# voidstrike/FPSG

Hardware: AMD Instinct MI355X
Metric: episodes/sec (+ Chamfer-kernel HBM GB/s in roofline.hbm), 2048-pt clouds, 224x224 images; episode = fwd + Chamfer + bwd, step = E episodes + all-reduce + Adam (higher is better)
Workload: dtype f32

## Files before the change

### fpsg_amd/_hip.py

```python
from __future__ import annotations

import ctypes
import os
import threading

import torch

_HERE = os.path.dirname(os.path.abspath(__file__))
LIB_PATH = os.environ.get("FPSG_HIP_LIB") or os.path.join(_HERE, "libfpsg_hip.so")

_c_f32p = ctypes.c_void_p
_c_i32p = ctypes.c_void_p
_c_int = ctypes.c_int
_c_stream = ctypes.c_void_p

SIGNATURES = {
    "fpsg_version": [],
    "fpsg_last_error": [],
    "fpsg_chamfer_fwd": [_c_f32p, _c_f32p, _c_int, _c_int, _c_int,
                         _c_f32p, _c_i32p, _c_f32p, _c_i32p, _c_stream],
    "fpsg_chamfer_bwd": [_c_f32p, _c_f32p, _c_i32p, _c_i32p, _c_f32p, _c_f32p,
                         _c_int, _c_int, _c_int, _c_f32p, _c_f32p, _c_stream],
    "fpsg_chamfer_losses": [_c_f32p, _c_f32p, _c_int, _c_int, _c_int, _c_int, ctypes.c_float, ctypes.c_float, _c_f32p,
                            _c_stream],
# ... 54 lines not shown
                         _c_int, _c_int, _c_int, _c_int, _c_f32p, _c_f32p, _c_f32p, _c_f32p, _c_f32p, _c_stream],
    "fpsg_bn_act_rows_fwd": [_c_f32p, _c_int, ctypes.POINTER(ctypes.c_int), ctypes.POINTER(ctypes.c_int), _c_int,
                             _c_f32p, _c_f32p, _c_f32p, _c_int, ctypes.c_float, _c_int, ctypes.c_float, _c_f32p,
                             _c_f32p, _c_f32p, _c_stream],
    "fpsg_bn_act_rows_bwd": [_c_f32p, _c_int, ctypes.POINTER(ctypes.c_int), ctypes.POINTER(ctypes.c_int), _c_int,
                             _c_f32p, _c_f32p, _c_f32p, _c_int, _c_int, ctypes.c_float, _c_f32p, _c_f32p, _c_f32p,
                             _c_f32p, _c_stream],
    "fpsg_bn_workspace_floats": [_c_int, _c_int, _c_int],
    "fpsg_bn_act_fwd": [_c_f32p, _c_f32p, _c_f32p, _c_f32p, _c_f32p, _c_f32p, ctypes.c_float, _c_int, _c_int, _c_int, _c_int,
                        ctypes.c_float, _c_int, ctypes.c_float, _c_f32p, _c_f32p, _c_f32p, _c_f32p, _c_f32p,
                        _c_stream],
    "fpsg_bn_act_bwd": [_c_f32p, _c_f32p, _c_f32p, _c_f32p, _c_int, _c_int, _c_int, _c_int, _c_int,
                        ctypes.c_float, _c_f32p, _c_f32p, _c_f32p, _c_f32p, _c_f32p, _c_f32p, _c_stream],
    "fpsg_bn_act_bwd_coef": [_c_f32p, _c_f32p, _c_f32p, _c_f32p, _c_int, _c_int, _c_int, _c_int, _c_int, ctypes.c_float,
                             _c_f32p, _c_f32p, _c_f32p, _c_f32p, _c_stream],
    "fpsg_bn_act_bwd_parts": [_c_f32p, _c_f32p, _c_f32p, _c_f32p, _c_int, _c_int, _c_int, _c_int, _c_int,
                        ctypes.c_float, _c_f32p, _c_f32p, _c_f32p, _c_f32p, _c_f32p, _c_f32p, _c_f32p, _c_int, _c_stream],
    "fpsg_bn_pool_workspace_floats": [_c_int, _c_int, _c_int, _c_int],
    "fpsg_bn_act_pool_fwd": [_c_f32p, _c_f32p, _c_f32p, _c_f32p, _c_f32p, _c_f32p, ctypes.c_float, _c_int, _c_int, _c_int, _c_int,
                             _c_int, ctypes.c_float, _c_int, ctypes.c_float, _c_f32p, _c_f32p, _c_f32p, _c_f32p,
                             _c_f32p, _c_f32p, _c_int, _c_stream],
    "fpsg_bn_act_pool_bwd": [_c_f32p, _c_f32p, _c_f32p, _c_f32p, _c_int, _c_int, _c_int, _c_int, _c_int, _c_int,
                             ctypes.c_float, _c_f32p, _c_f32p, _c_f32p, _c_f32p, _c_f32p, _c_f32p, _c_stream],
    "fpsg_bn_max_workspace_floats": [_c_int, _c_int, _c_int],
    "fpsg_bn_max_dz_offset": [_c_int, _c_int, _c_int],
    "fpsg_bn_act_max_fwd": [_c_f32p, _c_f32p, _c_f32p, _c_f32p, _c_f32p, _c_f32p, ctypes.c_float, _c_int, _c_int, _c_int, _c_int,
                            ctypes.c_float, _c_int, ctypes.c_float, _c_f32p, _c_i32p, _c_f32p, _c_f32p, _c_f32p,
                            _c_f32p, _c_stream],
    "fpsg_bn_act_max_bwd": [_c_f32p, _c_f32p, _c_f32p, _c_i32p, _c_f32p, _c_int, _c_int, _c_int, _c_int, _c_int,
                            ctypes.c_float, _c_f32p, _c_f32p, _c_f32p, _c_f32p, _c_f32p, _c_f32p, _c_stream],
# ... 17 lines not shown
    "fpsg_wino_output_transform_bwd_stats": [_c_int, _c_f32p, _c_int, _c_int, _c_int, _c_int, _c_f32p, _c_f32p, _c_f32p,
                                             _c_f32p, _c_f32p, ctypes.c_long, _c_stream],
    "fpsg_wino_filter_transform_batch": [ctypes.c_void_p, _c_int, ctypes.c_long, _c_stream],
    "fpsg_wino_filter_grad_transform": [_c_int, _c_f32p, _c_int, _c_int, _c_f32p, _c_stream],
    "fpsg_wino_conv_fused": [_c_f32p, _c_f32p, _c_int, _c_int, _c_int, _c_int, _c_int, _c_f32p, _c_stream],
    "fpsg_wino_input_transform_act": [_c_int, _c_f32p, _c_f32p, _c_f32p, _c_int, _c_int, _c_int, _c_int, _c_f32p, ctypes.c_long,
                                      _c_stream],
    "fpsg_wino_conv_fused_act": [_c_f32p, _c_f32p, _c_f32p, _c_f32p, _c_int, _c_int, _c_int, _c_int, _c_int, _c_f32p,
                                 _c_stream],
    "fpsg_wino_dw_fused_workspace_floats": [_c_int, _c_int, _c_int, _c_int],
    "fpsg_wino_dw_fused": [_c_f32p, _c_f32p, _c_f32p, _c_f32p, _c_int, _c_int, _c_int, _c_int, _c_int, _c_f32p, _c_f32p,
                           _c_stream],
    "fpsg_wino_conv_fused_parts": [_c_int, _c_int, _c_int, _c_int],
    "fpsg_wino_conv_fused_stats": [_c_f32p, _c_f32p, _c_f32p, _c_f32p, _c_int, _c_int, _c_int, _c_int, _c_int, _c_f32p,
                                   _c_f32p, _c_f32p, _c_stream],
    "fpsg_bn_stats": [_c_f32p, _c_f32p, _c_f32p, _c_f32p, _c_f32p, _c_f32p, ctypes.c_float, _c_int, _c_int, _c_int, _c_int,
                      ctypes.c_float, _c_f32p, _c_f32p, _c_f32p, _c_f32p, _c_f32p, _c_int, _c_stream],
    "fpsg_conv_first_dw_workspace_floats": [_c_int, _c_int, _c_int],
    "fpsg_conv_first_parts": [_c_int, _c_int, _c_int],
    "fpsg_conv_first_fwd": [_c_f32p, _c_f32p, _c_int, _c_int, _c_int, _c_int, _c_int, _c_f32p, _c_f32p, _c_f32p, _c_stream],
    "fpsg_conv_first_dw": [_c_f32p, _c_f32p, _c_int, _c_int, _c_int, _c_int, _c_int, _c_f32p, _c_f32p, _c_stream],
    "fpsg_conv_first_dw_fold": [_c_f32p, _c_f32p, _c_f32p, _c_f32p, _c_f32p, _c_f32p, _c_int, _c_int, _c_int, _c_int, _c_int,
                                _c_f32p, _c_f32p, _c_stream],
    "fpsg_adam_step": [_c_f32p, _c_f32p, _c_f32p, _c_f32p, ctypes.c_size_t, ctypes.c_float, ctypes.c_float,
                       ctypes.c_float, ctypes.c_float, _c_int, ctypes.c_float, _c_stream],
    "fpsg_flat_accumulate_segments": [_c_f32p, ctypes.c_void_p, ctypes.c_void_p, _c_int, ctypes.c_size_t, _c_int, _c_stream],
    "fpsg_flat_accumulate_tables": [_c_f32p, ctypes.c_void_p, ctypes.c_void_p, _c_int, _c_int, ctypes.c_size_t, _c_int,
                                    _c_stream],
    "fpsg_adam_step_segments": [_c_f32p, ctypes.c_void_p, ctypes.c_void_p, _c_int, _c_f32p, _c_f32p, ctypes.c_size_t,
                                ctypes.c_float, ctypes.c_float, ctypes.c_float, ctypes.c_float, _c_int, ctypes.c_float,
# ... 90 lines not shown
```

### fpsg_amd/csrc/bnact.hip

```cpp
#include <algorithm>
#include <atomic>
#include <cstdlib>

#include "fpsg_common.h"

namespace fpsg {
namespace {

constexpr int kBnThreads = 256;
constexpr int kBnSeg = 4096;
constexpr int kBnSlices = 64;
constexpr int kBnU = kBnSeg / 4 / kBnThreads;

enum BnAct { kActNone = 0, kActRelu = 1, kActLeaky = 2 };

template <int ACT>
__device__ __forceinline__ float act_fwd(float z, float slope) {
  if (ACT == kActRelu) return z > 0.0f ? z : 0.0f;
  if (ACT == kActLeaky) return z > 0.0f ? z : z * slope;
  return z;
}
template <int ACT>
__device__ __forceinline__ float act_grad(float z, float slope) {
  if (ACT == kActRelu) return z > 0.0f ? 1.0f : 0.0f;
// ... 376 lines not shown
                a0 += dz[u];
                a1 = fma_rn(dz[u], (xv[u] - mu) * rs, a1);
              }
              if (keep) sd[(size_t)n * L4 + e0] = dz;
            }
            if (keep) sx[(size_t)n * L4 + e0] = xv;
          }
        }
      }
    }
    for (int n = n_first; n < N; n += rpi) {
      const size_t base = ((size_t)n * C + c) * ld;
      if (vec) {
        const v4f* __restrict__ xp = reinterpret_cast<const v4f*>(x + base);
        const v4f* __restrict__ gp = reinterpret_cast<const v4f*>(MODE == 1 ? dy + base : x + base);
        for (int e = e0; e < L4; e += tpr) {
          v4f xv = xp[e];
#pragma unroll
          for (int u = 0; u < 4; ++u) xv[u] += b;
          if (MODE == 0) {
#pragma unroll
            for (int u = 0; u < 4; ++u) { a0 += xv[u]; a1 = fma_rn(xv[u], xv[u], a1); }
          } else {
            const v4f gv = gp[e];
            v4f dz;
#pragma unroll
            for (int u = 0; u < 4; ++u) {
              dz[u] = gv[u] * act_grad<ACT>(fma_rn(xv[u], sc, sh), slope);
              a0 += dz[u];
              a1 = fma_rn(dz[u], (xv[u] - mu) * rs, a1);
            }
            if (keep) sd[(size_t)n * L4 + e] = dz;
          }
          if (keep) sx[(size_t)n * L4 + e] = xv;
        }
      } else {
        for (int e = e0; e < L; e += tpr) {
          const float xv = x[base + e] + b;
          if (MODE == 0) {
            a0 += xv; a1 = fma_rn(xv, xv, a1);
          } else {
            const float dz = dy[base + e] * act_grad<ACT>(fma_rn(xv, sc, sh), slope);
            a0 += dz; a1 = fma_rn(dz, (xv - mu) * rs, a1);
          }
        }
      }
    }
    block_reduce2(a0, a1, red);
    if (threadIdx.x == 0) {
// ... 21 lines not shown
    }
    __syncthreads();
    if (MODE == 0) { sc = bc[0]; sh = bc[1]; }
  } else {
    if (threadIdx.x == 0) { bc[0] = sc; bc[1] = 0.0f; bc[2] = 0.0f; }
    __syncthreads();
  }
  const float k1 = bc[0], k2 = bc[1], k3 = bc[2];
  float acc = 0.0f, unused = 0.0f;
  for (int n = n0; n < N; n += rpi) {
    const size_t base = ((size_t)n * C + c) * ld;
    if (vec) {
      const v4f* __restrict__ xp = reinterpret_cast<const v4f*>(x + base);
      const v4f* __restrict__ gp = reinterpret_cast<const v4f*>(MODE == 1 ? dy + base : x + base);
      v4f* __restrict__ op = reinterpret_cast<v4f*>(out + base);
      for (int e = e0; e < L4; e += tpr) {
        v4f xv;
        if (keep) {
          xv = sx[(size_t)n * L4 + e];
        } else {
          xv = xp[e];
#pragma unroll
          for (int u = 0; u < 4; ++u) xv[u] += b;
        }
        v4f r;
        if (MODE == 0) {
#pragma unroll
          for (int u = 0; u < 4; ++u) r[u] = act_fwd<ACT>(fma_rn(xv[u], sc, sh), slope);
        } else {
          v4f dz;
          if (keep) {
            dz = sd[(size_t)n * L4 + e];
          } else {
            const v4f gv = gp[e];
#pragma unroll
            for (int u = 0; u < 4; ++u) dz[u] = gv[u] * act_grad<ACT>(fma_rn(xv[u], sc, sh), slope);
          }
#pragma unroll
          for (int u = 0; u < 4; ++u) r[u] = fma_rn(k1, dz[u], fma_rn(k2, xv[u], k3));
          acc += (r[0] + r[1]) + (r[2] + r[3]);
        }
        op[e] = r;
      }
    } else {
      for (int e = e0; e < L; e += tpr) {
        const float xv = x[base + e] + b;
        if (MODE == 0) {
          out[base + e] = act_fwd<ACT>(fma_rn(xv, sc, sh), slope);
        } else {
          const float dz = dy[base + e] * act_grad<ACT>(fma_rn(xv, sc, sh), slope);
          const float r = fma_rn(k1, dz, fma_rn(k2, xv, k3));
          out[base + e] = r;
          acc += r;
        }
      }
    }
  }
// ... 667 lines not shown
  int rc = check_dims("fpsg_bn_act_bwd_coef", N, C, L, act);
  if (rc) return rc;
  FPSG_REQUIRE_PTR(x); FPSG_REQUIRE_PTR(dy); FPSG_REQUIRE_PTR(chan);
  FPSG_REQUIRE_PTR(dgamma); FPSG_REQUIRE_PTR(dbeta); FPSG_REQUIRE_PTR(coef); FPSG_REQUIRE_PTR(ws);
  FPSG_REQUIRE(((reinterpret_cast<uintptr_t>(x) | reinterpret_cast<uintptr_t>(dy)) & 15) == 0, FPSG_E_ALIGN,
               "fpsg_bn_act_bwd_coef: x and dy must be 16-byte aligned");
  FPSG_REQUIRE((long)N * L > kBnSmallMax, FPSG_E_LIMIT, "fpsg_bn_act_bwd_coef: N*L = %ld is a small tensor (<= %d): use fpsg_bn_act_bwd",
               (long)N * L, kBnSmallMax);
  hipStream_t s = static_cast<hipStream_t>(stream);
  const int S = slices_for(N, L);
  launch_reduce<1>(act, x, dy, chan, pre_bias, N, C, L, S, slope, ws, s);
  if ((rc = launch_status("fpsg_bn_act_bwd_coef(reduce)"))) return rc;
  hipLaunchKernelGGL(bn_bwd_finalize_kernel, dim3(C), dim3(64), 0, s, ws, chan, C, S,
                     (double)N * (double)L, training, dgamma, dbeta, coef);
  return launch_status("fpsg_bn_act_bwd_coef(finalize)");
}

extern "C" int fpsg_bn_act_bwd_parts(const float* x, const float* pre_bias, const float* dy, const float* chan, int N,
                                     int C, int L, int training, int act, float slope, float* dx, float* dgamma,
                                     float* dbeta, float* dpre_bias, float* coef, float* ws, const float* parts,
                                     int n_parts, fpsg_stream_t stream) {
  using namespace fpsg;
  int rc = check_dims("fpsg_bn_act_bwd_parts", N, C, L, act);
  if (rc) return rc;
  FPSG_REQUIRE_PTR(x); FPSG_REQUIRE_PTR(dy); FPSG_REQUIRE_PTR(chan); FPSG_REQUIRE_PTR(dx); FPSG_REQUIRE_PTR(parts);
  FPSG_REQUIRE_PTR(dgamma); FPSG_REQUIRE_PTR(dbeta); FPSG_REQUIRE_PTR(coef);
  FPSG_REQUIRE(n_parts > 0, FPSG_E_SHAPE, "fpsg_bn_act_bwd_parts: n_parts must be positive (got %d)", n_parts);
  FPSG_REQUIRE(dpre_bias == nullptr || ws != nullptr, FPSG_E_NULL, "fpsg_bn_act_bwd_parts: dpre_bias needs the workspace");
  FPSG_REQUIRE(((reinterpret_cast<uintptr_t>(x) | reinterpret_cast<uintptr_t>(dy) | reinterpret_cast<uintptr_t>(dx)) & 15) == 0,
               FPSG_E_ALIGN, "fpsg_bn_act_bwd_parts: x, dy and dx must be 16-byte aligned");
// ... 195 lines not shown
```

### fpsg_amd/csrc/winograd_fused.hip

```cpp
#include <type_traits>

#include "fpsg_common.h"

namespace fpsg {
namespace {

constexpr int kFusedThreads = 256;
constexpr int kSteps = 16;
constexpr int kUldsFloats = 36 * kSteps * 64;

__device__ __forceinline__ float from_left_or(float keep, float v) {
  return __int_as_float(__builtin_amdgcn_update_dpp(__float_as_int(keep), __float_as_int(v), 0x111, 0xF, 0xF, false));
}
__device__ __forceinline__ float from_right_or(float keep, float v) {
  return __int_as_float(__builtin_amdgcn_update_dpp(__float_as_int(keep), __float_as_int(v), 0x101, 0xF, 0xF, false));
}
__device__ __forceinline__ void in4(const float (&d)[6], float c0, float (&t)[6]) {
  const float p = fma_rn(-4.0f, d[2], d[4]), q = fma_rn(-4.0f, d[1], d[3]);
  const float r = d[4] - d[2], s = d[3] - d[1];
  t[0] = fma_rn(c0, d[0], fma_rn(-5.0f, d[2], d[4]));
  t[1] = p + q;
  t[2] = p - q;
  t[3] = fma_rn(2.0f, s, r);
  t[4] = fma_rn(-2.0f, s, r);
  t[5] = fma_rn(4.0f, d[1], fma_rn(-5.0f, d[3], d[5]));
}
__device__ __forceinline__ void out4(const float (&m)[6], float (&s)[4]) {
  const float p12 = m[1] + m[2], m12 = m[1] - m[2], p34 = m[3] + m[4], m34 = m[3] - m[4];
  s[0] = (m[0] + p12) + p34;
  s[1] = fma_rn(2.0f, m34, m12);
  s[2] = fma_rn(4.0f, p34, p12);
  s[3] = fma_rn(8.0f, m34, m12) + m[5];
}

template <bool ACT, bool STATS, bool NT = false>
__global__ __launch_bounds__(kFusedThreads) void wino4_fused_c64_kernel(const float* __restrict__ x,
                                                                        const float* __restrict__ U ,
                                                                        int K, int H, int W, int Th, int Tw, long P,
                                                                        int S, float* __restrict__ y,
                                                                        const float* __restrict__ chan,
                                                                        const float* __restrict__ pre_bias,
                                                                        const float* __restrict__ out_bias,
                                                                        float* __restrict__ parts) {
  extern __shared__ __attribute__((aligned(16))) float ulds[];
  constexpr int C = 64;
  float* actp = ulds + kUldsFloats;
  const int tid = threadIdx.x, lane = tid & 63, wave = tid >> 6;
  const int kk = lane >> 4, col = lane & 15;
  const int i = blockIdx.x;
  const int slice = (i >> 3) % S;
  const int j = (i & 7) + 8 * (i / (8 * S));
  const int per_slice = gridDim.x / S;
  const int k0 = slice * 16;
  {
    const int kl = tid >> 4, c4 = tid & 15;
    const float* up = U + ((size_t)k0 + kl) * C + 4 * c4;
    v4f ub[36];
#pragma unroll
    for (int xi = 0; xi < 36; ++xi) ub[xi] = *reinterpret_cast<const v4f*>(up + (size_t)xi * K * C);
#pragma unroll
    for (int kq = 0; kq < 4; ++kq) {
      v4f* dst = reinterpret_cast<v4f*>(ulds + ((size_t)c4 * 64 + kq * 16 + kl) * 36);
#pragma unroll
      for (int x4 = 0; x4 < 9; ++x4)
        dst[x4] = (v4f){ub[4 * x4][kq], ub[4 * x4 + 1][kq], ub[4 * x4 + 2][kq], ub[4 * x4 + 3][kq]};
    }
  }
  if (ACT && tid < C) {
    actp[tid] = chan[tid];
    actp[C + tid] = chan[C + tid];
    actp[2 * C + tid] = pre_bias ? pre_bias[tid] : 0.0f;
  }
  __syncthreads();
  const __amdgpu_buffer_rsrc_t xrsrc = __builtin_amdgcn_make_buffer_rsrc(
      const_cast<float*>(x), 0, (int)(P * 16 * C * sizeof(float)), 0x00020000);
  float st0[4] = {0.0f, 0.0f, 0.0f, 0.0f}, st1[4] = {0.0f, 0.0f, 0.0f, 0.0f}, ob[4] = {0.0f, 0.0f, 0.0f, 0.0f};
  if (STATS && out_bias) {
#pragma unroll
    for (int r = 0; r < 4; ++r) ob[r] = out_bias[k0 + 4 * kk + r];
  }
  const long G = (P + 15) >> 4;
  struct Tile {
    uint32_t boff[6], eoffb[6];
    float c4t, mb, c4l, mr, mr5;
    int tw, th;
    unsigned n;
// ... 139 lines not shown
#pragma unroll 1
    for (int c4 = 2; c4 < kSteps - 2; c4 += 2) {
      FPSG_COMPUTE(c4, ra);
      FPSG_LOAD(c4 + 2, ra);
      FPSG_COMPUTE(c4 + 1, rb);
      FPSG_LOAD(c4 + 3, rb);
    }
    FPSG_COMPUTE(kSteps - 2, ra);
    FPSG_LOAD_NEXT(0, ra);
    FPSG_COMPUTE(kSteps - 1, rb);
    FPSG_LOAD_NEXT(1, rb);
#undef FPSG_COMPUTE
#undef FPSG_COMPUTE_FIRST
#undef FPSG_LOAD_NEXT
#undef FPSG_LOAD
    asm volatile("s_nop 15\n\ts_nop 15" ::: "memory");
    __builtin_amdgcn_sched_barrier(0);
#pragma unroll
    for (int r = 0; r < 4; ++r) {
      float s[6][4];
#pragma unroll
      for (int c = 0; c < 6; ++c) {
        float m[6];
#pragma unroll
        for (int a = 0; a < 6; ++a) m[a] = acc[6 * a + c][r];
        out4(m, s[c]);
      }
      if (live) {
        float* yp = y + ((((size_t)n * K + k0 + 4 * kk + r) * H) + 4 * th) * W + 4 * tw;
#pragma unroll
        for (int a = 0; a < 4; ++a) {
          float rowv[6], o[4];
#pragma unroll
          for (int c = 0; c < 6; ++c) rowv[c] = s[c][a];
          out4(rowv, o);
          st_stream<NT>(reinterpret_cast<v4f*>(yp + (size_t)a * W), (v4f){o[0], o[1], o[2], o[3]});
          if (STATS) {
#pragma unroll
            for (int u = 0; u < 4; ++u) {
              const float v = o[u] + ob[r];
              st0[r] += v;
              st1[r] = fma_rn(v, v, st1[r]);
            }
          }
        }
      }
    }
    cur = nxt;
  }
  if (STATS) {
    __syncthreads();
#pragma unroll
// ... 21 lines not shown
}

}
}

static long wino_fused_per_slice(long P, int S) {
  const long G = (P + 15) / 16;
  long per_slice = (256 + S - 1) / S;
  const long need = (G + 3) / 4;
  if (per_slice > need) per_slice = need;
  return ((per_slice + 7) / 8) * 8;
}

static int wino_conv_fused_launch(const char* fn, const float* x, const float* chan, const float* pre_bias,
                                  const float* U, int N, int C, int K, int H, int W, float* y, const float* out_bias,
                                  float* parts, fpsg_stream_t stream) {
  using namespace fpsg;
  FPSG_REQUIRE(C == 64, FPSG_E_SHAPE, "%s: C must be 64 (got %d)", fn, C);
  FPSG_REQUIRE(N > 0 && K > 0 && K % 16 == 0 && K <= 1024 && H > 0 && W > 0 && H % 4 == 0 && W % 4 == 0, FPSG_E_SHAPE,
               "%s: K a positive multiple of 16 (<= 1024), H and W positive multiples of 4 "
               "(got K=%d H=%d W=%d)", fn, K, H, W);
  FPSG_REQUIRE_PTR(x); FPSG_REQUIRE_PTR(U); FPSG_REQUIRE_PTR(y);
  FPSG_REQUIRE(((reinterpret_cast<uintptr_t>(x) | reinterpret_cast<uintptr_t>(y) | reinterpret_cast<uintptr_t>(U)) & 15) == 0,
               FPSG_E_ALIGN, "%s: x, y and U must be 16-byte aligned", fn);
  FPSG_REQUIRE(!misaligned4(out_bias) && !misaligned4(parts), FPSG_E_ALIGN, "%s: out_bias / parts not 4-byte aligned", fn);
  FPSG_REQUIRE((size_t)N * C * H * W * sizeof(float) < ((size_t)1 << 32), FPSG_E_LIMIT,
               "%s: x must be below 4 GiB (32-bit lane offsets; got N=%d H=%d W=%d)", fn, N, H, W);
  const long P = (long)N * (H / 4) * (W / 4);
  const int S = K / 16;
  const size_t lds_bytes = (size_t)(kUldsFloats + 3 * 64) * sizeof(float);
  typedef void (*kern_t)(const float*, const float*, int, int, int, int, int, long, int, float*, const float*,
                         const float*, const float*, float*);
  const bool nt = beyond_cache((size_t)N * K * H * W * sizeof(float));
  const kern_t kern =
      nt ? (chan ? (parts ? wino4_fused_c64_kernel<true, true, true> : wino4_fused_c64_kernel<true, false, true>)
                 : (parts ? wino4_fused_c64_kernel<false, true, true> : wino4_fused_c64_kernel<false, false, true>))
         : (chan ? (parts ? wino4_fused_c64_kernel<true, true> : wino4_fused_c64_kernel<true, false>)
                 : (parts ? wino4_fused_c64_kernel<false, true> : wino4_fused_c64_kernel<false, false>));
  const hipError_t lds_optin = hipFuncSetAttribute(reinterpret_cast<const void*>(kern),
                                                   hipFuncAttributeMaxDynamicSharedMemorySize, 160 * 1024);
  if (lds_optin != hipSuccess) {
    set_error("%s: cannot reserve %zu B of LDS: %s", fn, lds_bytes, hipGetErrorString(lds_optin));
    return static_cast<int>(lds_optin);
  }
  dim3 grid((unsigned)(wino_fused_per_slice(P, S) * S));
  hipLaunchKernelGGL(kern, grid, dim3(kFusedThreads), lds_bytes, static_cast<hipStream_t>(stream), x, U, K, H, W, H / 4,
                     W / 4, P, S, y, chan, pre_bias, out_bias, parts);
  return launch_status(fn);
}

extern "C" int fpsg_wino_conv_fused(const float* x, const float* U, int N, int C, int K, int H, int W, float* y,
                                    fpsg_stream_t stream) {
  return wino_conv_fused_launch("fpsg_wino_conv_fused", x, nullptr, nullptr, U, N, C, K, H, W, y, nullptr, nullptr, stream);
}

extern "C" int fpsg_wino_conv_fused_act(const float* x, const float* chan, const float* pre_bias, const float* U,
                                        int N, int C, int K, int H, int W, float* y, fpsg_stream_t stream) {
  using namespace fpsg;
  FPSG_REQUIRE_PTR(chan);
  FPSG_REQUIRE(!misaligned4(pre_bias), FPSG_E_ALIGN, "fpsg_wino_conv_fused_act: pre_bias not 4-byte aligned");
  return wino_conv_fused_launch("fpsg_wino_conv_fused_act", x, chan, pre_bias, U, N, C, K, H, W, y, nullptr, nullptr, stream);
}

extern "C" int fpsg_wino_conv_fused_parts(int N, int K, int H, int W) {
  if (N <= 0 || K <= 0 || K % 16 || H <= 0 || W <= 0 || H % 4 || W % 4) return 0;
  return (int)wino_fused_per_slice((long)N * (H / 4) * (W / 4), K / 16);
}

extern "C" int fpsg_wino_conv_fused_stats(const float* x, const float* chan, const float* pre_bias, const float* U,
                                          int N, int C, int K, int H, int W, float* y, const float* out_bias,
                                          float* parts, fpsg_stream_t stream) {
  using namespace fpsg;
  FPSG_REQUIRE_PTR(parts);
  FPSG_REQUIRE(!misaligned4(pre_bias), FPSG_E_ALIGN, "fpsg_wino_conv_fused_stats: pre_bias not 4-byte aligned");
  return wino_conv_fused_launch("fpsg_wino_conv_fused_stats", x, chan, pre_bias, U, N, C, K, H, W, y, out_bias, parts, stream);
}
```

### fpsg_amd/winograd.py

```python
from __future__ import annotations

import os

import torch

from . import _hip, gemm_split
from .bn_counters import count_batch

MIN_CHANNELS_M4 = 64
MIN_CHANNELS_M2 = 128
MIN_WIDE_CHANNELS_M2 = 256


def enabled() -> bool:
    return os.environ.get("FPSG_WINOGRAD", "1") != "0"


def _eligible_layer(conv: torch.nn.Conv2d, H: int, W: int) -> bool:
    def is_(v, want):
        return v == want or v == (want, want)
    return (enabled() and is_(conv.kernel_size, 3) and is_(conv.stride, 1) and is_(conv.padding, 1) and is_(conv.dilation, 1)
            and conv.groups == 1 and conv.padding_mode == "zeros" and H % 2 == 0 and W % 2 == 0
            and _wide_enough(conv.in_channels, conv.out_channels, tile_size(H, W)))

# ... 308 lines not shown
    parts = torch.empty((K, S, 2), dtype=torch.float32, device=x.device)
    opt = lambda t: _hip.ptr(t) if t is not None else None
    _call("fpsg_wino_conv_fused_stats", _hip.ptr(x), opt(chan), opt(pre_bias), _hip.ptr(U), N, C, K, H, W, _hip.ptr(y),
          opt(stats_bias), _hip.ptr(parts), _hip.stream_of(x))
    return y, parts


def _fused(x, U):
    N, C, H, W = x.shape
    K = U.shape[1]
    y = torch.empty((N, K, H, W), dtype=torch.float32, device=x.device)
    _call("fpsg_wino_conv_fused", _hip.ptr(x), _hip.ptr(U), N, C, K, H, W, _hip.ptr(y), _hip.stream_of(x))
    return y


def _grad_output(m, gy):
    N, K, H, W = gy.shape
    Ps = row_stride(N * _tiles(H, W, m))
    dM = torch.empty(((m + 2) ** 2, K, Ps), dtype=torch.float32, device=gy.device)
    _call("fpsg_wino_grad_output_transform", m, _hip.ptr(gy), N, K, H, W, _hip.ptr(dM), Ps, _hip.stream_of(gy))
    return dM


def grad_transforms_enabled() -> bool:
    return os.environ.get("FPSG_GRAD_TRANSFORMS", "1") != "0"


def _grad_transforms(m, gy):
    N, K, H, W = gy.shape
    Ps = row_stride(N * _tiles(H, W, m))
# ... 145 lines not shown
            return (None,) * 14
        y, chan, pre_bias, w, V = ctx.saved_tensors
        N, C, H, W, m, training, has_g, has_b = ctx.cfg
        K = w.shape[0]
        lib = _hip.load()
        dev = y.device
        gout = gout.contiguous()
        gw = None
        with torch.cuda.device(dev):
            bwd_parts = None
            fuse_dx = _can_fuse(m, K, C, N * H * W, H, W)
            fuse_dw = V is None and _can_fuse_dw(m, C, K, N, H, W)
            Vg = dM = None
            if ctx.needs_input_grad[9] and not fuse_dx and not fuse_dw and grad_transforms_enabled():
                Vg, dM = _grad_transforms(m, gout)
            if fuse_dx:
                ga = _fused(gout, _filter(m, w, True))
            elif bwd_stats_enabled() and N * H * W > _BN_SMALL_MAX:
                ga, bwd_parts = _output_bwd_stats(m, _bmm(_filter(m, w, True), Vg if Vg is not None else _input(m, gout)),
                                                  N, H, W, y, pre_bias, chan)
            else:
                ga = _output(m, _bmm(_filter(m, w, True), Vg if Vg is not None else _input(m, gout)), N, H, W)
            Vg = None
            if ctx.needs_input_grad[9]:
                if fuse_dw:
                    gw = _filter_grad(m, _fused_dw(y, chan, pre_bias, gout), w)
                else:
                    if V is None:
                        V = _input_act(m, y, chan, pre_bias)
                    gw = _filter_grad(m, _bmm_nt(dM if dM is not None else _grad_output(m, gout), V), w)
            want_dpb = pre_bias is not None and ctx.needs_input_grad[1]
# ... 61 lines not shown
            ctx.mark_non_differentiable(out_parts)
        return out, out_parts

    @staticmethod
    def backward(ctx, gout, _gparts=None):
        if gout is None:
            return (None,) * 13
        x, w1, y1, chan, b1, w2, V = ctx.saved_tensors
        N, C, H, W, m, has_g, has_b = ctx.cfg
        K = w2.shape[0]
        lib = _hip.load()
        dev = y1.device
        gout = gout.contiguous()
        gw1 = gw2 = db1 = None
        with torch.cuda.device(dev):
            if _can_fuse(m, K, C, N * H * W, H, W):
                ga = _fused(gout, _filter(m, w2, True))
            else:
                ga = _output(m, _bmm(_filter(m, w2, True), _input(m, gout)), N, H, W)
            if ctx.needs_input_grad[9]:
                if V is None and _can_fuse_dw(m, C, K, N, H, W):
                    gw2 = _filter_grad(m, _fused_dw(y1, chan, b1, gout), w2)
                else:
                    if V is None:
                        V = _input_act(m, y1, chan, b1)
                    gw2 = _filter_grad(m, _bmm_nt(_grad_output(m, gout), V), w2)
            dgamma = torch.empty((C,), dtype=torch.float32, device=dev)
            dbeta = torch.empty((C,), dtype=torch.float32, device=dev)
            coef = torch.empty((3, C), dtype=torch.float32, device=dev)
            ws = torch.empty((lib.fpsg_bn_workspace_floats(N, C, H * W),), dtype=torch.float32, device=dev)
            _call("fpsg_bn_act_bwd_coef", _hip.ptr(y1), _hip.ptr(b1), _hip.ptr(ga), _hip.ptr(chan), N, C, H * W, 1, 1, 0.0,
                  _hip.ptr(dgamma), _hip.ptr(dbeta), _hip.ptr(coef), _hip.ptr(ws), _hip.stream_of(y1))
            if ctx.needs_input_grad[1]:
                gw1 = torch.empty_like(w1, memory_format=torch.contiguous_format)
                ws1 = torch.empty((lib.fpsg_conv_first_dw_workspace_floats(N, H, W),), dtype=torch.float32, device=dev)
                xc = x.contiguous()
                _call("fpsg_conv_first_dw_fold", _hip.ptr(xc), _hip.ptr(y1), _hip.ptr(ga), _hip.ptr(chan), _hip.ptr(coef),
                      _hip.ptr(b1), N, 3, 64, H, W, _hip.ptr(gw1), _hip.ptr(ws1), _hip.stream_of(y1))
            if ctx.needs_input_grad[2]:
                db1 = torch.zeros((C,), dtype=torch.float32, device=dev)
        return (None, gw1, db1, dgamma if has_g else None, dbeta if has_b else None, None, None, None, None, gw2, None,
                None, None)


def stem_applies(x, conv1, bn1, conv2) -> bool:
    from . import conv_first
    if not (stem_fold_enabled() and fold_enabled() and bn1.training and bn1.track_running_stats and stats_enabled()):
# ... 39 lines not shown
```

### include/fpsg_hip.h

```cpp
#ifndef FPSG_HIP_H
#define FPSG_HIP_H

#include <stddef.h>
#include <stdint.h>

#ifdef __cplusplus
extern "C" {
#endif

typedef void* fpsg_stream_t;

#define FPSG_ABI_VERSION 1

#define FPSG_E_NULL   (-1)
#define FPSG_E_SHAPE  (-2)
#define FPSG_E_ALIGN  (-3)
#define FPSG_E_LIMIT  (-4)

int         fpsg_version(void);
const char* fpsg_last_error(void);

int fpsg_chamfer_fwd(const float* xyz1, const float* xyz2, int B, int N, int M,
                     float* dist1, int32_t* idx1, float* dist2, int32_t* idx2,
                     fpsg_stream_t stream);
// ... 139 lines not shown
size_t fpsg_bn_workspace_floats(int N, int C, int L);
int fpsg_bn_act_fwd(const float* x, const float* pre_bias, const float* gamma, const float* beta,
                    float* running_mean, float* running_var, float momentum, int N, int C, int L, int training,
                    float eps, int act, float slope, float* y, float* chan, float* batch_mean,
                    float* batch_var_unbiased, float* ws, fpsg_stream_t stream);
int fpsg_bn_stats(const float* x, const float* pre_bias, const float* gamma, const float* beta,
                  float* running_mean, float* running_var, float momentum, int N, int C, int L, int training,
                  float eps, float* chan, float* batch_mean, float* batch_var_unbiased, float* ws,
                  const float* parts, int n_parts, fpsg_stream_t stream);
int fpsg_bn_act_bwd(const float* x, const float* pre_bias, const float* dy, const float* chan, int N, int C,
                    int L, int training, int act, float slope, float* dx, float* dgamma, float* dbeta,
                    float* dpre_bias, float* coef, float* ws, fpsg_stream_t stream);
int fpsg_bn_act_bwd_coef(const float* x, const float* pre_bias, const float* dy, const float* chan, int N, int C,
                         int L, int training, int act, float slope, float* dgamma, float* dbeta, float* coef,
                         float* ws, fpsg_stream_t stream);
int fpsg_bn_act_rows_fwd(const float* x, int ld, const int* seg_off, const int* seg_len, int nseg,
                         const float* pre_bias, const float* gamma, const float* beta, int C, float eps, int act,
                         float slope, float* y, float* chan, float* stats, fpsg_stream_t stream);
int fpsg_bn_act_rows_bwd(const float* x, int ld, const int* seg_off, const int* seg_len, int nseg,
                         const float* pre_bias, const float* dy, const float* chan, int C, int act, float slope,
                         float* dx, float* dgamma, float* dbeta, float* dpre_bias, fpsg_stream_t stream);
int fpsg_bn_act_bwd_parts(const float* x, const float* pre_bias, const float* dy, const float* chan, int N,
                          int C, int L, int training, int act, float slope, float* dx, float* dgamma,
                          float* dbeta, float* dpre_bias, float* coef, float* ws, const float* parts,
                          int n_parts, fpsg_stream_t stream);

size_t fpsg_bn_pool_workspace_floats(int N, int C, int H, int W);
int fpsg_bn_act_pool_fwd(const float* x, const float* pre_bias, const float* gamma, const float* beta,
                         float* running_mean, float* running_var, float momentum, int N, int C, int H, int W,
                         int training, float eps, int act, float slope, float* y_pooled, float* chan,
// ... 59 lines not shown
int fpsg_gemm_split_nn_packed(const void* Ap, const float* B, float* C, int batch, int M, int N, int K, int ldb, int ldc,
                              long sB, long sC, int variant, fpsg_stream_t stream);

int fpsg_gemm_split_nn_persistent(const void* Ap, const float* B, float* C, int batch, int M, int N, int K, int ldb, int ldc,
                                  long sB, long sC, int variant, fpsg_stream_t stream);

int fpsg_gemm_f32_nn(const float* A, const float* B, float* C, int batch, int M, int N, int K, int lda, int ldb, int ldc,
                     long sA, long sB, long sC, int variant, fpsg_stream_t stream);

int fpsg_wino_conv_fused(const float* x, const float* U, int N, int C, int K, int H, int W, float* y,
                         fpsg_stream_t stream);

int fpsg_wino_conv_fused_parts(int N, int K, int H, int W);
int fpsg_wino_conv_fused_stats(const float* x, const float* chan, const float* pre_bias, const float* U, int N, int C,
                               int K, int H, int W, float* y, const float* out_bias, float* parts, fpsg_stream_t stream);

size_t fpsg_wino_dw_fused_workspace_floats(int N, int K, int H, int W);
int fpsg_wino_dw_fused(const float* x, const float* chan, const float* pre_bias, const float* dy, int N, int C, int K,
                       int H, int W, float* dU, float* ws, fpsg_stream_t stream);

int fpsg_wino_input_transform_act(int m, const float* x, const float* chan, const float* pre_bias, int N, int C,
                                  int H, int W, float* V, long ldp, fpsg_stream_t stream);
int fpsg_wino_conv_fused_act(const float* x, const float* chan, const float* pre_bias, const float* U, int N, int C,
                             int K, int H, int W, float* y, fpsg_stream_t stream);

size_t fpsg_conv_first_dw_workspace_floats(int N, int H, int W);
int fpsg_conv_first_dw(const float* x, const float* dy, int N, int C, int K, int H, int W, float* dw, float* ws,
                       fpsg_stream_t stream);
int fpsg_conv_first_dw_fold(const float* x, const float* y, const float* ga, const float* chan, const float* coef,
                            const float* pre_bias, int N, int C, int K, int H, int W, float* dw, float* ws,
// ... 20 lines not shown
```

Measured before the change: 46.00.

## Fuse BN backward statistics into Winograd fused dgrad epilogue

```diff
diff --git a/fpsg_amd/_hip.py b/fpsg_amd/_hip.py
--- a/fpsg_amd/_hip.py
+++ b/fpsg_amd/_hip.py
@@ -92,6 +92,8 @@
                         ctypes.c_float, _c_f32p, _c_f32p, _c_f32p, _c_f32p, _c_f32p, _c_f32p, _c_stream],
     "fpsg_bn_act_bwd_coef": [_c_f32p, _c_f32p, _c_f32p, _c_f32p, _c_int, _c_int, _c_int, _c_int, _c_int, ctypes.c_float,
                              _c_f32p, _c_f32p, _c_f32p, _c_f32p, _c_stream],
+    "fpsg_bn_act_bwd_coef_parts": [_c_f32p, _c_int, _c_int, _c_int, _c_int, _c_f32p, _c_f32p, _c_f32p, _c_f32p, _c_int,
+                                   _c_stream],
     "fpsg_bn_act_bwd_parts": [_c_f32p, _c_f32p, _c_f32p, _c_f32p, _c_int, _c_int, _c_int, _c_int, _c_int,
                         ctypes.c_float, _c_f32p, _c_f32p, _c_f32p, _c_f32p, _c_f32p, _c_f32p, _c_f32p, _c_int, _c_stream],
     "fpsg_bn_pool_workspace_floats": [_c_int, _c_int, _c_int, _c_int],
@@ -139,6 +141,8 @@
     "fpsg_wino_conv_fused_parts": [_c_int, _c_int, _c_int, _c_int],
     "fpsg_wino_conv_fused_stats": [_c_f32p, _c_f32p, _c_f32p, _c_f32p, _c_int, _c_int, _c_int, _c_int, _c_int, _c_f32p,
                                    _c_f32p, _c_f32p, _c_stream],
+    "fpsg_wino_conv_fused_bwd_stats": [_c_f32p, _c_f32p, _c_int, _c_int, _c_int, _c_int, _c_int, _c_f32p, _c_f32p, _c_f32p,
+                                       _c_f32p, _c_f32p, _c_stream],
     "fpsg_bn_stats": [_c_f32p, _c_f32p, _c_f32p, _c_f32p, _c_f32p, _c_f32p, ctypes.c_float, _c_int, _c_int, _c_int, _c_int,
                       ctypes.c_float, _c_f32p, _c_f32p, _c_f32p, _c_f32p, _c_f32p, _c_int, _c_stream],
     "fpsg_conv_first_dw_workspace_floats": [_c_int, _c_int, _c_int],
diff --git a/fpsg_amd/csrc/bnact.hip b/fpsg_amd/csrc/bnact.hip
--- a/fpsg_amd/csrc/bnact.hip
+++ b/fpsg_amd/csrc/bnact.hip
@@ -414,25 +414,40 @@
       if (vec) {
         const v4f* __restrict__ xp = reinterpret_cast<const v4f*>(x + base);
         const v4f* __restrict__ gp = reinterpret_cast<const v4f*>(MODE == 1 ? dy + base : x + base);
-        for (int e = e0; e < L4; e += tpr) {
-          v4f xv = xp[e];
-#pragma unroll
-          for (int u = 0; u < 4; ++u) xv[u] += b;
-          if (MODE == 0) {
-#pragma unroll
-            for (int u = 0; u < 4; ++u) { a0 += xv[u]; a1 = fma_rn(xv[u], xv[u], a1); }
-          } else {
-            const v4f gv = gp[e];
-            v4f dz;
-#pragma unroll
-            for (int u = 0; u < 4; ++u) {
-              dz[u] = gv[u] * act_grad<ACT>(fma_rn(xv[u], sc, sh), slope);
-              a0 += dz[u];
-              a1 = fma_rn(dz[u], (xv[u] - mu) * rs, a1);
+        for (int eb = e0; eb < L4; eb += kBnU * tpr) {
+          v4f xq[kBnU], gq[kBnU];
+#pragma unroll
+          for (int j = 0; j < kBnU; ++j) {
+            const int e = eb + j * tpr;
+            xq[j] = gq[j] = (v4f){0.0f, 0.0f, 0.0f, 0.0f};
+            if (e < L4) {
+              xq[j] = xp[e];
+              if (MODE == 1) gq[j] = gp[e];
             }
-            if (keep) sd[(size_t)n * L4 + e] = dz;
           }
-          if (keep) sx[(size_t)n * L4 + e] = xv;
+#pragma unroll
+          for (int j = 0; j < kBnU; ++j) {
+            const int e = eb + j * tpr;
+            if (e < L4) {
+              v4f xv = xq[j];
+#pragma unroll
+              for (int u = 0; u < 4; ++u) xv[u] += b;
+              if (MODE == 0) {
+#pragma unroll
+                for (int u = 0; u < 4; ++u) { a0 += xv[u]; a1 = fma_rn(xv[u], xv[u], a1); }
+              } else {
+                v4f dz;
+#pragma unroll
+                for (int u = 0; u < 4; ++u) {
+                  dz[u] = gq[j][u] * act_grad<ACT>(fma_rn(xv[u], sc, sh), slope);
+                  a0 += dz[u];
+                  a1 = fma_rn(dz[u], (xv[u] - mu) * rs, a1);
+                }
+                if (keep) sd[(size_t)n * L4 + e] = dz;
+              }
+              if (keep) sx[(size_t)n * L4 + e] = xv;
+            }
+          }
         }
       } else {
         for (int e = e0; e < L; e += tpr) {
@@ -484,33 +499,48 @@
       const v4f* __restrict__ xp = reinterpret_cast<const v4f*>(x + base);
       const v4f* __restrict__ gp = reinterpret_cast<const v4f*>(MODE == 1 ? dy + base : x + base);
       v4f* __restrict__ op = reinterpret_cast<v4f*>(out + base);
-      for (int e = e0; e < L4; e += tpr) {
-        v4f xv;
-        if (keep) {
-          xv = sx[(size_t)n * L4 + e];
-        } else {
-          xv = xp[e];
-#pragma unroll
-          for (int u = 0; u < 4; ++u) xv[u] += b;
-        }
-        v4f r;
-        if (MODE == 0) {
-#pragma unroll
-          for (int u = 0; u < 4; ++u) r[u] = act_fwd<ACT>(fma_rn(xv[u], sc, sh), slope);
-        } else {
-          v4f dz;
-          if (keep) {
-            dz = sd[(size_t)n * L4 + e];
-          } else {
-            const v4f gv = gp[e];
-#pragma unroll
-            for (int u = 0; u < 4; ++u) dz[u] = gv[u] * act_grad<ACT>(fma_rn(xv[u], sc, sh), slope);
+      for (int eb = e0; eb < L4; eb += kBnU * tpr) {
+        v4f xq[kBnU], gq[kBnU];
+#pragma unroll
+        for (int j = 0; j < kBnU; ++j) {
+          const int e = eb + j * tpr;
+          xq[j] = gq[j] = (v4f){0.0f, 0.0f, 0.0f, 0.0f};
+          if (e < L4) {
+            if (keep) {
+              xq[j] = sx[(size_t)n * L4 + e];
+              if (MODE == 1) gq[j] = sd[(size_t)n * L4 + e];
+            } else {
+              xq[j] = xp[e];
+              if (MODE == 1) gq[j] = gp[e];
+            }
           }
-#pragma unroll
-          for (int u = 0; u < 4; ++u) r[u] = fma_rn(k1, dz[u], fma_rn(k2, xv[u], k3));
-          acc += (r[0] + r[1]) + (r[2] + r[3]);
-        }
-        op[e] = r;
+        }
+#pragma unroll
+        for (int j = 0; j < kBnU; ++j) {
+          const int e = eb + j * tpr;
+          if (e < L4) {
+            v4f xv = xq[j];
+            if (!keep) {
+#pragma unroll
+              for (int u = 0; u < 4; ++u) xv[u] += b;
+            }
+            v4f r;
+            if (MODE == 0) {
+#pragma unroll
+              for (int u = 0; u < 4; ++u) r[u] = act_fwd<ACT>(fma_rn(xv[u], sc, sh), slope);
+            } else {
+              v4f dz = gq[j];
+              if (!keep) {
+#pragma unroll
+                for (int u = 0; u < 4; ++u) dz[u] = gq[j][u] * act_grad<ACT>(fma_rn(xv[u], sc, sh), slope);
+              }
+#pragma unroll
+              for (int u = 0; u < 4; ++u) r[u] = fma_rn(k1, dz[u], fma_rn(k2, xv[u], k3));
+              acc += (r[0] + r[1]) + (r[2] + r[3]);
+            }
+            op[e] = r;
+          }
+        }
       }
     } else {
       for (int e = e0; e < L; e += tpr) {
@@ -1208,6 +1238,20 @@
   hipLaunchKernelGGL(bn_bwd_finalize_kernel, dim3(C), dim3(64), 0, s, ws, chan, C, S,
                      (double)N * (double)L, training, dgamma, dbeta, coef);
   return launch_status("fpsg_bn_act_bwd_coef(finalize)");
+}
+
+extern "C" int fpsg_bn_act_bwd_coef_parts(const float* chan, int N, int C, int L, int training, float* dgamma,
+                                          float* dbeta, float* coef, const float* parts, int n_parts,
+                                          fpsg_stream_t stream) {
+  using namespace fpsg;
+  int rc = check_dims("fpsg_bn_act_bwd_coef_parts", N, C, L, kActRelu);
+  if (rc) return rc;
+  FPSG_REQUIRE_PTR(chan); FPSG_REQUIRE_PTR(parts);
+  FPSG_REQUIRE_PTR(dgamma); FPSG_REQUIRE_PTR(dbeta); FPSG_REQUIRE_PTR(coef);
+  FPSG_REQUIRE(n_parts > 0, FPSG_E_SHAPE, "fpsg_bn_act_bwd_coef_parts: n_parts must be positive (got %d)", n_parts);
+  hipLaunchKernelGGL(bn_bwd_finalize_kernel, dim3(C), dim3(64), 0, static_cast<hipStream_t>(stream), parts, chan, C,
+                     n_parts, (double)N * (double)L, training, dgamma, dbeta, coef);
+  return launch_status("fpsg_bn_act_bwd_coef_parts(finalize)");
 }
 
 extern "C" int fpsg_bn_act_bwd_parts(const float* x, const float* pre_bias, const float* dy, const float* chan, int N,
diff --git a/fpsg_amd/csrc/winograd_fused.hip b/fpsg_amd/csrc/winograd_fused.hip
--- a/fpsg_amd/csrc/winograd_fused.hip
+++ b/fpsg_amd/csrc/winograd_fused.hip
@@ -33,7 +33,7 @@
   s[3] = fma_rn(8.0f, m34, m12) + m[5];
 }
 
-template <bool ACT, bool STATS, bool NT = false>
+template <bool ACT, bool STATS, bool NT = false, bool BWD = false>
 __global__ __launch_bounds__(kFusedThreads) void wino4_fused_c64_kernel(const float* __restrict__ x,
                                                                         const float* __restrict__ U ,
                                                                         int K, int H, int W, int Th, int Tw, long P,
@@ -41,7 +41,9 @@
                                                                         const float* __restrict__ chan,
                                                                         const float* __restrict__ pre_bias,
                                                                         const float* __restrict__ out_bias,
-                                                                        float* __restrict__ parts) {
+                                                                        float* __restrict__ parts,
+                                                                        const float* __restrict__ xpre) {
+  static_assert(!BWD || (STATS && !ACT), "BWD delivers sums (STATS) and does not activate its input");
   extern __shared__ __attribute__((aligned(16))) float ulds[];
   constexpr int C = 64;
   float* actp = ulds + kUldsFloats;
@@ -70,6 +72,11 @@
     actp[tid] = chan[tid];
     actp[C + tid] = chan[C + tid];
     actp[2 * C + tid] = pre_bias ? pre_bias[tid] : 0.0f;
+  }
+  if (BWD && tid < 16) {
+#pragma unroll
+    for (int q = 0; q < 4; ++q) actp[16 * q + tid] = chan[(size_t)q * K + k0 + tid];
+    actp[64 + tid] = pre_bias ? pre_bias[k0 + tid] : 0.0f;
   }
   __syncthreads();
   const __amdgpu_buffer_rsrc_t xrsrc = __builtin_amdgcn_make_buffer_rsrc(
@@ -239,6 +246,17 @@
 #undef FPSG_COMPUTE_FIRST
 #undef FPSG_LOAD_NEXT
 #undef FPSG_LOAD
+    const float* xq0 = nullptr;
+    v4f xrow[4];
+    auto load_xpre = [&](int r) {
+#pragma unroll
+      for (int a = 0; a < 4; ++a)
+        xrow[a] = ld_stream<NT>(reinterpret_cast<const v4f*>(xq0 + ((size_t)r * H + a) * W));
+    };
+    if constexpr (BWD) {
+      xq0 = xpre + ((((size_t)n * K + k0 + 4 * kk) * H) + 4 * th) * W + 4 * tw;
+      load_xpre(0);
+    }
     asm volatile("s_nop 15\n\ts_nop 15" ::: "memory");
     __builtin_amdgcn_sched_barrier(0);
 #pragma unroll
@@ -250,6 +268,15 @@
 #pragma unroll
         for (int a = 0; a < 6; ++a) m[a] = acc[6 * a + c][r];
         out4(m, s[c]);
+      }
+      float bsc = 0.0f, bsh = 0.0f, bmu = 0.0f, brs = 0.0f, bpb = 0.0f;
+      v4f xr[4];
+      if constexpr (BWD) {
+        bsc = actp[4 * kk + r]; bsh = actp[16 + 4 * kk + r]; bmu = actp[32 + 4 * kk + r]; brs = actp[48 + 4 * kk + r];
+        bpb = actp[64 + 4 * kk + r];
+#pragma unroll
+        for (int a = 0; a < 4; ++a) xr[a] = xrow[a];
+        if (r < 3) load_xpre(r + 1);
       }
       if (live) {
         float* yp = y + ((((size_t)n * K + k0 + 4 * kk + r) * H) + 4 * th) * W + 4 * tw;
@@ -260,7 +287,15 @@
           for (int c = 0; c < 6; ++c) rowv[c] = s[c][a];
           out4(rowv, o);
           st_stream<NT>(reinterpret_cast<v4f*>(yp + (size_t)a * W), (v4f){o[0], o[1], o[2], o[3]});
-          if (STATS) {
+          if constexpr (BWD) {
+#pragma unroll
+            for (int u = 0; u < 4; ++u) {
+              const float xv = xr[a][u] + bpb;
+              const float dz = fma_rn(xv, bsc, bsh) > 0.0f ? o[u] : 0.0f;
+              st0[r] += dz;
+              st1[r] = fma_rn(dz, (xv - bmu) * brs, st1[r]);
+            }
+          } else if (STATS) {
 #pragma unroll
             for (int u = 0; u < 4; ++u) {
               const float v = o[u] + ob[r];
@@ -312,7 +347,7 @@
 
 static int wino_conv_fused_launch(const char* fn, const float* x, const float* chan, const float* pre_bias,
                                   const float* U, int N, int C, int K, int H, int W, float* y, const float* out_bias,
-                                  float* parts, fpsg_stream_t stream) {
+                                  float* parts, fpsg_stream_t stream, const float* xpre = nullptr) {
   using namespace fpsg;
   FPSG_REQUIRE(C == 64, FPSG_E_SHAPE, "%s: C must be 64 (got %d)", fn, C);
   FPSG_REQUIRE(N > 0 && K > 0 && K % 16 == 0 && K <= 1024 && H > 0 && W > 0 && H % 4 == 0 && W % 4 == 0, FPSG_E_SHAPE,
@@ -328,9 +363,10 @@
   const int S = K / 16;
   const size_t lds_bytes = (size_t)(kUldsFloats + 3 * 64) * sizeof(float);
   typedef void (*kern_t)(const float*, const float*, int, int, int, int, int, long, int, float*, const float*,
-                         const float*, const float*, float*);
+                         const float*, const float*, float*, const float*);
   const bool nt = beyond_cache((size_t)N * K * H * W * sizeof(float));
   const kern_t kern =
+      xpre ? (nt ? wino4_fused_c64_kernel<false, true, true, true> : wino4_fused_c64_kernel<false, true, false, true>) :
       nt ? (chan ? (parts ? wino4_fused_c64_kernel<true, true, true> : wino4_fused_c64_kernel<true, false, true>)
                  : (parts ? wino4_fused_c64_kernel<false, true, true> : wino4_fused_c64_kernel<false, false, true>))
          : (chan ? (parts ? wino4_fused_c64_kernel<true, true> : wino4_fused_c64_kernel<true, false>)
@@ -343,7 +379,7 @@
   }
   dim3 grid((unsigned)(wino_fused_per_slice(P, S) * S));
   hipLaunchKernelGGL(kern, grid, dim3(kFusedThreads), lds_bytes, static_cast<hipStream_t>(stream), x, U, K, H, W, H / 4,
-                     W / 4, P, S, y, chan, pre_bias, out_bias, parts);
+                     W / 4, P, S, y, chan, pre_bias, out_bias, parts, xpre);
   return launch_status(fn);
 }
 
@@ -373,3 +409,16 @@
   FPSG_REQUIRE(!misaligned4(pre_bias), FPSG_E_ALIGN, "fpsg_wino_conv_fused_stats: pre_bias not 4-byte aligned");
   return wino_conv_fused_launch("fpsg_wino_conv_fused_stats", x, chan, pre_bias, U, N, C, K, H, W, y, out_bias, parts, stream);
 }
+
+extern "C" int fpsg_wino_conv_fused_bwd_stats(const float* x, const float* U, int N, int C, int K, int H, int W, float* y,
+                                              const float* xpre, const float* pre_bias, const float* chan,
+                                              float* parts, fpsg_stream_t stream) {
+  using namespace fpsg;
+  FPSG_REQUIRE_PTR(xpre); FPSG_REQUIRE_PTR(chan); FPSG_REQUIRE_PTR(parts);
+  FPSG_REQUIRE((reinterpret_cast<uintptr_t>(xpre) & 15) == 0, FPSG_E_ALIGN,
+               "fpsg_wino_conv_fused_bwd_stats: xpre must be 16-byte aligned");
+  FPSG_REQUIRE(!misaligned4(pre_bias) && !misaligned4(chan), FPSG_E_ALIGN,
+               "fpsg_wino_conv_fused_bwd_stats: pre_bias / chan not 4-byte aligned");
+  return wino_conv_fused_launch("fpsg_wino_conv_fused_bwd_stats", x, chan, pre_bias, U, N, C, K, H, W, y, nullptr, parts,
+                                stream, xpre);
+}
diff --git a/fpsg_amd/winograd.py b/fpsg_amd/winograd.py
--- a/fpsg_amd/winograd.py
+++ b/fpsg_amd/winograd.py
@@ -346,6 +346,17 @@
     return y
 
 
+def _fused_bwd_stats(gy, U, xpre, pre_bias, chan):
+    N, C, H, W = gy.shape
+    K = U.shape[1]
+    y = torch.empty((N, K, H, W), dtype=torch.float32, device=gy.device)
+    S = _hip.load().fpsg_wino_conv_fused_parts(N, K, H, W)
+    parts = torch.empty((K, S, 2), dtype=torch.float32, device=gy.device)
+    _call("fpsg_wino_conv_fused_bwd_stats", _hip.ptr(gy), _hip.ptr(U), N, C, K, H, W, _hip.ptr(y), _hip.ptr(xpre),
+          _hip.ptr(pre_bias) if pre_bias is not None else None, _hip.ptr(chan), _hip.ptr(parts), _hip.stream_of(gy))
+    return y, parts
+
+
 def _grad_output(m, gy):
     N, K, H, W = gy.shape
     Ps = row_stride(N * _tiles(H, W, m))
@@ -521,7 +532,9 @@
             Vg = dM = None
             if ctx.needs_input_grad[9] and not fuse_dx and not fuse_dw and grad_transforms_enabled():
                 Vg, dM = _grad_transforms(m, gout)
-            if fuse_dx:
+            if fuse_dx and bwd_stats_enabled() and N * H * W > _BN_SMALL_MAX:
+                ga, bwd_parts = _fused_bwd_stats(gout, _filter(m, w, True), y, pre_bias, chan)
+            elif fuse_dx:
                 ga = _fused(gout, _filter(m, w, True))
             elif bwd_stats_enabled() and N * H * W > _BN_SMALL_MAX:
                 ga, bwd_parts = _output_bwd_stats(m, _bmm(_filter(m, w, True), Vg if Vg is not None else _input(m, gout)),
@@ -613,8 +626,12 @@
         gout = gout.contiguous()
         gw1 = gw2 = db1 = None
         with torch.cuda.device(dev):
+            bwd_parts = None
             if _can_fuse(m, K, C, N * H * W, H, W):
-                ga = _fused(gout, _filter(m, w2, True))
+                if bwd_stats_enabled():
+                    ga, bwd_parts = _fused_bwd_stats(gout, _filter(m, w2, True), y1, b1, chan)
+                else:
+                    ga = _fused(gout, _filter(m, w2, True))
             else:
                 ga = _output(m, _bmm(_filter(m, w2, True), _input(m, gout)), N, H, W)
             if ctx.needs_input_grad[9]:
@@ -627,9 +644,13 @@
             dgamma = torch.empty((C,), dtype=torch.float32, device=dev)
             dbeta = torch.empty((C,), dtype=torch.float32, device=dev)
             coef = torch.empty((3, C), dtype=torch.float32, device=dev)
-            ws = torch.empty((lib.fpsg_bn_workspace_floats(N, C, H * W),), dtype=torch.float32, device=dev)
-            _call("fpsg_bn_act_bwd_coef", _hip.ptr(y1), _hip.ptr(b1), _hip.ptr(ga), _hip.ptr(chan), N, C, H * W, 1, 1, 0.0,
-                  _hip.ptr(dgamma), _hip.ptr(dbeta), _hip.ptr(coef), _hip.ptr(ws), _hip.stream_of(y1))
+            if bwd_parts is not None:
+                _call("fpsg_bn_act_bwd_coef_parts", _hip.ptr(chan), N, C, H * W, 1, _hip.ptr(dgamma), _hip.ptr(dbeta),
+                      _hip.ptr(coef), _hip.ptr(bwd_parts), bwd_parts.shape[1], _hip.stream_of(y1))
+            else:
+                ws = torch.empty((lib.fpsg_bn_workspace_floats(N, C, H * W),), dtype=torch.float32, device=dev)
+                _call("fpsg_bn_act_bwd_coef", _hip.ptr(y1), _hip.ptr(b1), _hip.ptr(ga), _hip.ptr(chan), N, C, H * W, 1, 1,
+                      0.0, _hip.ptr(dgamma), _hip.ptr(dbeta), _hip.ptr(coef), _hip.ptr(ws), _hip.stream_of(y1))
             if ctx.needs_input_grad[1]:
                 gw1 = torch.empty_like(w1, memory_format=torch.contiguous_format)
                 ws1 = torch.empty((lib.fpsg_conv_first_dw_workspace_floats(N, H, W),), dtype=torch.float32, device=dev)
diff --git a/include/fpsg_hip.h b/include/fpsg_hip.h
--- a/include/fpsg_hip.h
+++ b/include/fpsg_hip.h
@@ -177,6 +177,8 @@
 int fpsg_bn_act_bwd_coef(const float* x, const float* pre_bias, const float* dy, const float* chan, int N, int C,
                          int L, int training, int act, float slope, float* dgamma, float* dbeta, float* coef,
                          float* ws, fpsg_stream_t stream);
+int fpsg_bn_act_bwd_coef_parts(const float* chan, int N, int C, int L, int training, float* dgamma, float* dbeta,
+                               float* coef, const float* parts, int n_parts, fpsg_stream_t stream);
 int fpsg_bn_act_rows_fwd(const float* x, int ld, const int* seg_off, const int* seg_len, int nseg,
                          const float* pre_bias, const float* gamma, const float* beta, int C, float eps, int act,
                          float slope, float* y, float* chan, float* stats, fpsg_stream_t stream);
@@ -266,6 +268,9 @@
 int fpsg_wino_conv_fused_parts(int N, int K, int H, int W);
 int fpsg_wino_conv_fused_stats(const float* x, const float* chan, const float* pre_bias, const float* U, int N, int C,
                                int K, int H, int W, float* y, const float* out_bias, float* parts, fpsg_stream_t stream);
+int fpsg_wino_conv_fused_bwd_stats(const float* x, const float* U, int N, int C, int K, int H, int W, float* y,
+                                   const float* xpre, const float* pre_bias, const float* chan, float* parts,
+                                   fpsg_stream_t stream);
 
 size_t fpsg_wino_dw_fused_workspace_floats(int N, int K, int H, int W);
 int fpsg_wino_dw_fused(const float* x, const float* chan, const float* pre_bias, const float* dy, int N, int C, int K,
```

Result: no change. 45.66 (median of 2 runs) (-0.7%).
